# jbrea/BayesianOptimization.jl

Hardware: AMD Instinct MI355X
Metric: acquisition-candidates/sec (N=3000,d=8) (higher is better)
Workload: dtype f64

## Files before the change

### bayesianoptimization.jl_amd/csrc/bohip.hip

```cpp
#include "../../include/bohip.h"
#include "../../include/bohip_paths.h"
#include "../../include/bohip_fit.h"
#include "../../include/bohip_qei.h"
#include "../../include/bohip_acq.h"
#include "../../include/bohip_kg.h"
#include "../../include/bohip_mes.h"
#include "../../include/bohip_ens.h"
#include "../../include/bohip_ens_grad.h"
#include "../../include/bohip_con.h"
#include "../../include/bohip_mo.h"
#include "../../include/bohip_loo.h"
#include "../../include/bohip_loo_batch.h"
#include "../../include/bohip_rep.h"
#include "kernels_linalg.hip"
#include "kernels_loo.hip"
#include "kernels_rep.hip"
#include "kernels_chol.hip"
#include "kernels_exec.hip"
#include "kernels_score.hip"
#include "kernels_batch.hip"
#include "kernels_sample.hip"
#include "kernels_qei.hip"
#include "kernels_kg.hip"
#include "kernels_mes.hip"
// ... 307 lines not shown
    for (DBuf<double>* b : {&g->dX, &g->dy, &g->dL, &g->dW, &g->dWT, &g->dS, &g->dalpha, &g->dr, &g->dt, &g->dApp, &g->dchol_idl}) b->release();
    g->dchol_flags.release();
    g->dinvr.release();
    g->ex_T = 0;
    return 0;
}
static size_t chol_flag_words(int T);
static size_t chol_abort_word(int T);
static int upload_site_weights(bohip_gp* g) {
    HIPCHK(g->dinvr.reserve(std::max<size_t>(1, (size_t)std::max(g->cap, g->n)), g->stream));
    if (g->n > 0) HIPCHK(hipMemcpyAsync(g->dinvr, g->hinvr.data(), (size_t)g->n * 8, hipMemcpyHostToDevice, g->stream));
    return 0;
}
static int refuse_weighted(const bohip_gp* g, const char* who) {
    if (!g || !g->weighted) return 0;
    return fail(BOHIP_E_UNSUPPORTED, std::string(who) + " does not support a model with replicated sites (bohip_gp_append_sites with reps > 1): "
                                         "its kernels build the covariance with one noise term for every row");
}
static int alloc_model(bohip_gp* g, int64_t cap) {
    free_model(g);
    for (DBuf<double>* b : {&g->dKsT, &g->dVT, &g->dUT, &g->dq, &g->dBV}) b->release();
    g->kst_rows = 0;
    g->cap = cap;
    g->ld = round_up(cap + 1, TILE) + 16;
    const size_t ld = (size_t)g->ld, mat = ld * ld * sizeof(double);
    hipStream_t st = g->stream;
    HIPCHK(g->dX.reserve(std::max<size_t>(1, (size_t)cap * g->d), st));
    HIPCHK(g->dy.reserve(std::max<size_t>(1, (size_t)cap), st));
    for (DBuf<double>* b : {&g->dL, &g->dW, &g->dWT, &g->dS}) HIPCHK(b->reserve(ld * ld, st));
    for (DBuf<double>* b : {&g->dalpha, &g->dr, &g->dt}) HIPCHK(b->reserve(ld + 256, st));
    HIPCHK(g->dApp.reserve((size_t)APP_ROWS * ld, st));
    {
        const size_t Tm = (size_t)(g->ld / TILE) + 1;
        HIPCHK(g->dchol_flags.reserve(chol_flag_words((int)std::min<size_t>(Tm, CHOL_DF_TCAP)), st));
        HIPCHK(g->dchol_idl.reserve(Tm * CH_PANELS * 256, st));
    }
    HIPCHK(hipMemsetAsync(g->dL, 0, mat, g->stream));
    HIPCHK(hipMemsetAsync(g->dW, 0, mat, g->stream));
    HIPCHK(hipMemsetAsync(g->dWT, 0, mat, g->stream));
    HIPCHK(hipMemsetAsync(g->dS, 0, mat, g->stream));
    if (g->n > 0) {
        HIPCHK(hipMemcpyAsync(g->dX, g->hX.data(), (size_t)g->n * g->d * 8, hipMemcpyHostToDevice, g->stream));
        HIPCHK(hipMemcpyAsync(g->dy, g->hy.data(), (size_t)g->n * 8, hipMemcpyHostToDevice, g->stream));
    }
    if (g->weighted) CHK(upload_site_weights(g));
    g->stale = true;
    return 0;
}

static int g_bulk_pieces = 4;
static int g_sample_mfma_min = 200;
static int g_path_mfma_min = 24;
static int g_split = 1;
static int g_asc_wg_nmax = 256;
static const double g_asc_first_step = 0.1;
static int g_asc_fold = 1;
static int g_asc_lockstep = 0;
static int g_small_m = 0;
static int g_small_r = -1;
static int g_inv_hi_h = 16;
static int g_chol_df = 1;
static bool g_chol_df_strict = false;
static bool g_chol_df_dump = false;
static int g_chol_df_tmax = 96;
static std::atomic<int> g_chol_df_skip{0}, g_chol_df_backoff{0};
static unsigned long long g_chol_spin_ticks = CH_SPIN_TICKS_DEFAULT;
static int g_chol_exec_patience_us = 1000;
static int g_chol_exec_fill_inv = 1;
static int g_chol_exec_inv_pairs = 0;
static std::atomic<int> g_chol_inv_grp_min{28};
static std::atomic<int> g_chol_inv_g{8};
static int g_chol_nsf = 3;
static int g_chol_exec_urgent = -1;
static int g_chol_exec_second = 1;
static int g_small_zero_copy = 1;
static int g_chol_exec_nbu = 2;
static int g_chol_exec_fast = -1;
static int g_chol_exec_pairs = -1;
static int g_chol_exec_wgs = -1;
static int g_append_alpha_inc = 1;
static int64_t g_chunk_rows_forced = 0;
static int g_prune_m = -1;
static int g_pa_order = 1;
static int launch_gemm_nt(bohip_gp* g, const GemmNTParams& p, int batch = 1, hipStream_t st = nullptr, bool hi = false) {
    if (p.mt <= 0 || p.nt64 <= 0 || p.kc <= 0 || batch <= 0) return 0;
    if (hi) hipLaunchKernelGGL(k_gemm_nt_hi, dim3(p.mt * p.nt64, batch), dim3(GEMM_THREADS_8), glds3_lds_bytes<4>(), st ? st : g->stream, p);
    else hipLaunchKernelGGL(k_gemm_nt, dim3(p.mt * p.nt64, batch), dim3(GEMM_THREADS_8), glds3_lds_bytes<4>(), st ? st : g->stream, p);
    HIPCHK(hipGetLastError());
    return 0;
}

static int device_cus();
static void read_dev_knobs() {
#if BOHIP_DEV_KNOBS
    struct Knob { const char* name; int* v; int lo, hi; };
    static int chunk_rows = 0, dump = 0;
    const Knob knobs[] = {
        {"BOHIP_CHOL_DF_TMAX", &g_chol_df_tmax, 0, CHOL_DF_TCAP}, {"BOHIP_INV_HI_H", &g_inv_hi_h, 0, 1 << 20},
        {"BOHIP_CHOL_EXEC_PAIRS", &g_chol_exec_pairs, -1, 64},
        {"BOHIP_CHOL_EXEC_URGENT", &g_chol_exec_urgent, 1, 1 << 20}, {"BOHIP_CHOL_NSF", &g_chol_nsf, 1, CH_NSF_MAX},
        {"BOHIP_CHOL_EXEC_PATIENCE_US", &g_chol_exec_patience_us, 0, 1 << 30}, {"BOHIP_CHOL_EXEC_FILL_INV", &g_chol_exec_fill_inv, 0, 1},
        {"BOHIP_CHOL_EXEC_INV_PAIRS", &g_chol_exec_inv_pairs, 0, 1}, {"BOHIP_CHOL_EXEC_WGS", &g_chol_exec_wgs, 1, 1 << 20},
        {"BOHIP_CHOL_EXEC_FAST", &g_chol_exec_fast, -1, 1 << 20},
        {"BOHIP_CHOL_EXEC_SECOND", &g_chol_exec_second, 0, 1}, {"BOHIP_SMALL_ZERO_COPY", &g_small_zero_copy, 0, 1}, {"BOHIP_CHOL_EXEC_NBU", &g_chol_exec_nbu, 0, 16}, {"BOHIP_CHUNK_ROWS", &chunk_rows, 0, 1 << 30},
        {"BOHIP_PRUNE_M", &g_prune_m, -1, 1 << 16}, {"BOHIP_PA_ORDER", &g_pa_order, 0, 1},
        {"BOHIP_APPEND_ALPHA_INC", &g_append_alpha_inc, 0, 1}, {"BOHIP_BULK_PIECES", &g_bulk_pieces, 0, 8}, {"BOHIP_SPLIT", &g_split, 0, 1},
        {"BOHIP_SMALL_R", &g_small_r, 0, SMALL_MAX}, {"BOHIP_SMALL_M", &g_small_m, 0, 1 << 20}, {"BOHIP_CHOL_DF_DUMP", &dump, 0, 1},
    };
    for (const Knob& k : knobs)
        if (const char* e = getenv(k.name)) *k.v = std::min(k.hi, std::max(k.lo, atoi(e)));
    g_chunk_rows_forced = chunk_rows;
    g_chol_df_dump = dump != 0;
#endif
}

template <class Setup>
static int once_per_device(bool (&done)[64], int device, Setup&& setup) {
    if (done[device & 63]) return 0;
    CHK(setup());
    done[device & 63] = true;
    return 0;
}

static int kernel_setup_of_this_device() {
    HIPCHK(hipFuncSetAttribute((const void*)k_potf2_inv, hipFuncAttributeMaxDynamicSharedMemorySize, POTF2_LDS_BYTES));
    HIPCHK(hipFuncSetAttribute((const void*)k_gemm_nt, hipFuncAttributeMaxDynamicSharedMemorySize, glds3_lds_bytes<4>()));
    HIPCHK(hipFuncSetAttribute((const void*)k_trigemm_sq, hipFuncAttributeMaxDynamicSharedMemorySize, glds3_lds_bytes<4>()));
    HIPCHK(hipFuncSetAttribute((const void*)k_trigemm_sq_pa, hipFuncAttributeMaxDynamicSharedMemorySize, glds3_lds_bytes<4>()));
    HIPCHK(hipFuncSetAttribute((const void*)k_trigemm_rows, hipFuncAttributeMaxDynamicSharedMemorySize, RS_LDS_BYTES));
    HIPCHK(hipFuncSetAttribute((const void*)k_batch_cond<true>, hipFuncAttributeMaxDynamicSharedMemorySize, BATCH_LDS_MAX));
    HIPCHK(hipFuncSetAttribute((const void*)k_batch_cond<false>, hipFuncAttributeMaxDynamicSharedMemorySize, BATCH_LDS_MAX));
    HIPCHK(hipFuncSetAttribute((const void*)k_chol_chain, hipFuncAttributeMaxDynamicSharedMemorySize, CH_LDS_BYTES));
    HIPCHK(hipFuncSetAttribute((const void*)k_gemm_nt_hi, hipFuncAttributeMaxDynamicSharedMemorySize, glds3_lds_bytes<4>()));
    HIPCHK(hipFuncSetAttribute((const void*)k_chol_exec, hipFuncAttributeMaxDynamicSharedMemorySize, glds3_lds_bytes<4>()));
    HIPCHK(hipFuncSetAttribute((const void*)k_trimv_stream<TRIMV_D>, hipFuncAttributeMaxDynamicSharedMemorySize, trimv_lds_bytes(TRIMV_D)));
    HIPCHK(hipFuncSetAttribute((const void*)k_path_mfma<true>, hipFuncAttributeMaxDynamicSharedMemorySize, (int)path_mfma_lds_bytes(DMAX)));
    HIPCHK(hipFuncSetAttribute((const void*)k_path_mfma<false>, hipFuncAttributeMaxDynamicSharedMemorySize, (int)path_mfma_lds_bytes(DMAX)));
    HIPCHK(hipFuncSetAttribute((const void*)k_kg<true>, hipFuncAttributeMaxDynamicSharedMemorySize, (int)kg_lds_bytes(KG_RMAX)));
    HIPCHK(hipFuncSetAttribute((const void*)k_kg<false>, hipFuncAttributeMaxDynamicSharedMemorySize, (int)kg_lds_bytes(KG_RMAX)));
    if (const char* e = getenv("BOHIP_CHOL_DATAFLOW")) g_chol_df = atoi(e);
    if (const char* e = getenv("BOHIP_CHOL_SPIN_US")) g_chol_spin_ticks = 100ull * (unsigned long long)std::max(1, atoi(e));
    if (const char* e = getenv("BOHIP_CHOL_INV_G")) g_chol_inv_g = std::min(64, std::max(0, atoi(e)));
    if (const char* e = getenv("BOHIP_CHOL_INV_GRP_MIN")) g_chol_inv_grp_min = std::max(0, atoi(e));
    if (const char* e = getenv("BOHIP_ASC_WG_NMAX")) g_asc_wg_nmax = std::max(0, atoi(e));
    if (const char* e = getenv("BOHIP_ASC_LOCKSTEP")) { g_asc_lockstep = atoi(e) == 1; g_asc_fold = atoi(e) != 2; }
    if (const char* e = getenv("BOHIP_SAMPLE_MFMA_MIN")) g_sample_mfma_min = std::max(1, atoi(e));
    g_chol_df_strict = getenv("BOHIP_CHOL_DF_STRICT") != nullptr;
    read_dev_knobs();
    return 0;
}
static int one_time_kernel_setup() {
    static bool done[64] = {false};
    int dev = 0;
    HIPCHK(hipGetDevice(&dev));
    return once_per_device(done, dev, kernel_setup_of_this_device);
}

static int launch_rows_trimv(bohip_gp* g, const double* W, int64_t N0, const double* rows, int P, double* out, int upper);
static int compute_alpha(bohip_gp* g) {
    const int64_t N = g->n;
    g->alpha_inc_run = 0;
    hipLaunchKernelGGL(k_sub_mean, dim3((N + 255) / 256), dim3(256), 0, g->stream, g->dy, g->beta, N, g->dr);
    HIPCHK(hipGetLastError());
    CHK(launch_rows_trimv(g, g->dW, N, g->dr, 1, g->dt, 0));
    CHK(launch_rows_trimv(g, g->dWT, N, g->dt, 1, g->dalpha, 1));
    HIPCHK(hipMemcpyAsync(g->dW + N * g->ld, g->dalpha, (size_t)N * 8, hipMemcpyDeviceToDevice, g->stream));
    return 0;
}

static int check_info(bohip_gp* g) {
    int local = 0;
    int* const pw = g->hpin ? g->pin.words + 1 : &local;
    HIPCHK(hipMemcpyAsync(pw, g->dinfo, sizeof(int), hipMemcpyDeviceToHost, g->stream));
    HIPCHK(hipStreamSynchronize(g->stream));
    const int info = *pw;
    if (info != 0) {
        g->pivot = info;
        g->stale = true;
        return fail(BOHIP_E_NOTPD, "kernel matrix not positive definite at pivot " + std::to_string(info));
    }
    g->pivot = 0;
    return 0;
}

static int inverse_level(bohip_gp* g, hipStream_t st, int t0, int nt, int h) {
    const int64_t ld = g->ld, base = (int64_t)t0 * TILE * (ld + 1);
    const int pairs = (nt + 2 * h - 1) / (2 * h);
    const int64_t zs = (int64_t)2 * h * TILE * (ld + 1);
// ... 841 lines not shown
    if (grew) HIPCHK(hipMemsetAsync(g->dVT, 0, n * 8, g->stream));
    return 0;
}
static int ensure_xs(bohip_gp* g, int64_t R) {
    HIPCHK(g->dXs.reserve(std::max<size_t>(1, (size_t)R * g->d), g->stream));
    return 0;
}

struct PassDims { int64_t N, Npad, R, Rpad, ld; int T; };
static int row_tiles(const bohip_gp* g) { return (int)(round_up(g->n + 1, TILE) / TILE); }
static PassDims pass_dims(const bohip_gp* g, int64_t R) {
    const int T = row_tiles(g);
    return PassDims{g->n, (int64_t)T * TILE, R, round_up(R, TILE) + TILE, g->ld, T};
}
struct SplitPlan { int kz = 0, nsl = 0; };
enum class Route { Small, Split, Pruned, WholeK };
struct PassPlan {
    PassDims dm{};
    Route route = Route::WholeK;
    SplitPlan sp;
    int prune_m = 0;
    int64_t chunk = 0;
    int dq_tiles() const { return route == Route::WholeK || route == Route::Pruned ? dm.T : 0; }
};

template <int DT>
static void launch_kstar(bohip_gp* g, const double* dXs, int64_t r0, int64_t r1, int64_t Npad, const KernelHyper& hp, const KstarParts* kp) {
    const int rb = r1 - r0 <= 32 && !kp ? 2 : 16;
    dim3 grid((Npad + 255) / 256, (r1 - r0 + rb - 1) / rb);
    if (kp)
        LAUNCH_FAM(fam_low(hp), (k_kstar<DT, true, true>), (k_kstar<DT, false, true>), grid, dim3(256), 0, g->stream, g->dX, g->n, Npad, dXs,
                   r0, r1, hp, g->dKsT, g->ld, rb, *kp);
    else
        LAUNCH_FAM(fam_low(hp), (k_kstar<DT, true>), (k_kstar<DT, false>), grid, dim3(256), 0, g->stream, g->dX, g->n, Npad, dXs, r0, r1, hp,
                   g->dKsT, g->ld, rb, KstarParts{});
}

static void trigemm_pieces(int T, int64_t alpha_row, std::vector<int>& out) {
    struct P { double cost; int code; };
    std::vector<P> ps;
    for (int rt = 0; rt < T; ++rt) {
        const int64_t live = alpha_row + 1 - (int64_t)rt * TILE;
        if (live <= TILE / 2) ps.push_back({(rt + 0.5) / 2.0, rt | PIECE_UPPER_SOLO << 16});
        else ps.push_back({rt + 1.0, rt | PIECE_WHOLE << 16});
    }
    std::stable_sort(ps.begin(), ps.end(), [](const P& a, const P& b) { return a.cost > b.cost; });
    out.clear();
    for (const P& q : ps) out.push_back(q.code);
}
static int ensure_pieces(bohip_gp* g, int T, int64_t alpha_row) {
    if (g->pieces_T == T && g->pieces_alpha == alpha_row && g->dpieces) return 0;
    std::vector<int> ps;
    trigemm_pieces(T, alpha_row, ps);
    if (T > 65535) return fail(BOHIP_E_UNSUPPORTED, "too many row tiles");
    if (ps.size() > g->dpieces.capacity()) HIPCHK(g->dpieces.reserve(2 * ps.size() + 64, g->stream));
    g->hpieces = ps;
    HIPCHK(hipMemcpyAsync(g->dpieces, g->hpieces.data(), ps.size() * sizeof(int), hipMemcpyHostToDevice, g->stream));
    g->n_pieces = (int)ps.size();
    g->pieces_T = T; g->pieces_alpha = alpha_row;
    return 0;
}

static int ensure_clk(bohip_gp* g) {
    bool grew = false;
    HIPCHK(g->dclk.reserve(2, g->stream, Grow::Exact, &grew));
    if (grew) HIPCHK(hipMemsetAsync(g->dclk, 0, 2 * sizeof(unsigned long long), g->stream));
    return 0;
}
static int launch_trigemm(bohip_gp* g, const PassDims& dm, int64_t r0, int64_t ncand, double* VT, FuseParams fz) {
    const int CT = (int)((ncand + CTILE - 1) / CTILE), n_local = (CT + 7) / 8;
    CHK(ensure_pieces(g, dm.T, dm.N));
    const int NP = g->n_pieces;
    fz.T = dm.T;
    if (g->timing) {
        CHK(ensure_clk(g));
        fz.clk = g->dclk;
    }
    hipLaunchKernelGGL(k_trigemm_sq, dim3(8 * n_local * NP), dim3(GEMM_THREADS_8), glds3_lds_bytes<4>(), g->stream, g->dW, g->ld,
                       g->dKsT, g->ld, g->dpieces, NP, CT, dm.N, g->dq, dm.Rpad, g->dmu_raw, r0, VT, g->ld, fz);
    HIPCHK(hipGetLastError());
    return 0;
}

static int launch_kstar_any(bohip_gp* g, const double* dXs, int64_t r0, int64_t r1, int64_t Npad, const KernelHyper& hp,
                            const KstarParts* kp = nullptr) {
    dispatch_dt(g->d, [&](auto dt) { launch_kstar<decltype(dt)::value>(g, dXs, r0, r1, Npad, hp, kp); });
    HIPCHK(hipGetLastError());
    return 0;
}

static int launch_gemm_u(bohip_gp* g, const PassDims& dm, int CT) {
    GemmNTParams p{};
    p.A = g->dVT; p.lda = dm.ld; p.B = g->dWT; p.ldb = dm.ld; p.C = g->dUT; p.ldc = dm.ld;
    p.mt = CT; p.nt64 = 2 * dm.T; p.kc = dm.T * (TILE / KC); p.alpha = 1.0; p.beta = 0.0; p.klo_from_n = 1;
    return launch_gemm_nt(g, p);
}

struct ChunkV { double* VT = nullptr; int64_t row_stride = 0; };
template <class Finish>
static int64_t chunk_pass(bohip_gp* g, const PassPlan& pl, const double* dXs, const KernelHyper& hp, ChunkV v, bool want_u, const FuseParams& fz, Finish&& finish) {
    const PassDims& dm = pl.dm;
    int64_t chunks = 0;
    for (int64_t r0 = 0; r0 < dm.R; r0 += pl.chunk, ++chunks) {
        const int64_t r1 = std::min(dm.R, r0 + pl.chunk);
        t_begin(g, "kstar");
        CHK(launch_kstar_any(g, dXs, r0, r1, dm.Npad, hp));
        t_end(g);
        t_begin(g, v.VT ? "trigemm_sq+V" : "trigemm_sq");
        CHK(launch_trigemm(g, dm, r0, r1 - r0, v.VT ? v.VT + r0 * v.row_stride : nullptr, fz));
        t_end(g);
        if (want_u) {
            t_begin(g, "gemm_U");
            CHK(launch_gemm_u(g, dm, (int)((r1 - r0 + TILE - 1) / TILE)));
            t_end(g);
        }
        CHK(finish(r0, r1));
    }
    return chunks;
}
static int no_finish(int64_t, int64_t) { return 0; }

static int ensure_small_counters(bohip_gp* g) {
    bool grew = false;
    HIPCHK(g->dgparts.reserve((size_t)SMALL_MAX * 16 * (2 * DMAX), g->stream));
    HIPCHK(g->dgcount.reserve(SMALL_MAX, g->stream, Grow::Exact, &grew));
    if (grew) HIPCHK(hipMemsetAsync(g->dgcount, 0, SMALL_MAX * sizeof(unsigned), g->stream));
    return 0;
}
static bool split_applicable(const bohip_gp* g);
static int64_t small_limit(const bohip_gp* g) {
    if (g_small_r >= 0) return g_small_r;
    if (split_applicable(g)) return std::min<int64_t>(SMALL_MAX, std::max<int64_t>(16, (20 + 260000 / std::max<int64_t>(g->n, 1)) / 16 * 16));
    return std::min<int64_t>(SMALL_MAX, 90 + 300000 / std::max<int64_t>(g->n, 1));
}
static int64_t path_R(const bohip_gp* g, int64_t R) { return std::max(R, g->batch_hint); }
#ifdef BOHIP_SMALL_TRACE
static unsigned long long* g_small_trace = nullptr;
extern "C" int bohip_debug_small_trace_read(unsigned long long* out) {
    if (!g_small_trace) return -1;
    return hipMemcpy(out, g_small_trace, 8192 * 16 * 8, hipMemcpyDeviceToHost) == hipSuccess ? 0 : -2;
}
#endif
template <int DT, int G>
static void launch_small_pass(bohip_gp* g, const SmallCommon& sc, const SmallCommon& scu, const SmallV& sv, const SmallU* su, const KernelHyper& hp,
                              int npass) {
    const bool lo = fam_low(hp);
    LAUNCH_FAM(lo, (k_small_v<DT, G, true>), (k_small_v<DT, G, false>), dim3((unsigned)sc.ntiles, (unsigned)npass), dim3(SP_THREADS), 0,
               g->stream, sc, sv, hp);
    if (su) {
        if (DT == 64 && su->sv.ap.acq == ACQ_LOGEI)
            LAUNCH_FAM(lo, (k_small_u_logei64<true>), (k_small_u_logei64<false>), dim3((unsigned)sc.ntiles, (unsigned)npass), dim3(SP_THREADS), 0,
                       g->stream, scu, *su, hp);
        else
            LAUNCH_FAM(lo, (k_small_u<DT, G, true>), (k_small_u<DT, G, false>), dim3((unsigned)sc.ntiles, (unsigned)npass), dim3(SP_THREADS), 0,
                       g->stream, scu, *su, hp);
    }
}
template <int DT>
static void launch_small_pass_g(bohip_gp* g, int G, const SmallCommon& sc, const SmallCommon& scu, const SmallV& sv, const SmallU* su,
                                const KernelHyper& hp, int npass) {
    if constexpr (DT <= 16) {
        if (G == 1) return launch_small_pass<DT, 1>(g, sc, scu, sv, su, hp, npass);
        if (G == 2) return launch_small_pass<DT, 2>(g, sc, scu, sv, su, hp, npass);
        if (G == 3) return launch_small_pass<DT, 3>(g, sc, scu, sv, su, hp, npass);
    }
    launch_small_pass<DT, 4>(g, sc, scu, sv, su, hp, npass);
}
struct AscPass {
    const SmallFold* fold = nullptr;
// ... 144 lines not shown
    std::stable_sort(out.begin(), out.end(), [](int a, int b) {
        return 8 * (a & 0xffff) + ((a >> 16) & 1) * 4 > 8 * (b & 0xffff) + ((b >> 16) & 1) * 4;
    });
    return out;
}
static int rows_halves_from(const std::vector<int>& hv, int t0) {
    int n = 0;
    while (n < (int)hv.size() && (hv[n] & 0xffff) >= t0) ++n;
    return n;
}
static int launch_trigemm_rows(bohip_gp* g, const double* KsT, const int* halves, int NH, const int* list, const unsigned* cnt,
                               int cnt_max, double* q, int64_t ldq, double* mu, int groups = 0, const PruneFinish* pf = nullptr,
                               unsigned* arrive = nullptr) {
    if (NH <= 0 || cnt_max <= 0) return 0;
    RowsParams rp{};
    rp.W = g->dW; rp.ldw = g->ld; rp.KsT = KsT; rp.ldk = g->ld; rp.list = list; rp.cnt = cnt; rp.cnt_max = cnt_max;
    rp.halves = halves; rp.NH = NH; rp.G = groups > 0 ? groups : (cnt_max + RS_COLS - 1) / RS_COLS;
    rp.alpha_row = g->n; rp.q = q; rp.ldq = ldq; rp.mu = mu;
    if (pf) { rp.finish = 1; rp.arrive = arrive; rp.pf = *pf; }
    hipLaunchKernelGGL(k_trigemm_rows, dim3((unsigned)(8 * ((NH + 7) / 8) * rp.G)), dim3(RS_THREADS), RS_LDS_BYTES, g->stream, rp);
    HIPCHK(hipGetLastError());
    return 0;
}
static int launch_trigemm_on(bohip_gp* g, const double* KsT, const int* pieces, int NP, int CT, double* q, int64_t ldq, double* mu_raw,
                             FuseParams fz) {
    const int n_local = (CT + 7) / 8;
    if (NP <= 0 || CT <= 0) return 0;
    if (g->timing && g->dclk) fz.clk = g->dclk;
    hipLaunchKernelGGL(k_trigemm_sq, dim3(8 * n_local * NP), dim3(GEMM_THREADS_8), glds3_lds_bytes<4>(), g->stream, g->dW, g->ld, KsT,
                       g->ld, pieces, NP, CT, g->n, q, ldq, mu_raw, (int64_t)0, nullptr, g->ld, fz);
    HIPCHK(hipGetLastError());
    return 0;
}
static std::vector<int> phase_a_jobs(const std::vector<int>& pieces, int m) {
    std::vector<int> out;
    for (int c : pieces)
        if ((c & 0xffff) < m) { out.push_back((c & 0xffff) | 1 << 16); out.push_back(c & 0xffff); }
    std::stable_sort(out.begin(), out.end(), [](int a, int b) {
        return 8 * (a & 0xffff) + (a >> 16) * 4 > 8 * (b & 0xffff) + (b >> 16) * 4;
    });
    if (g_pa_order == 1) std::rotate(out.begin(), out.begin() + out.size() / 3, out.begin() + 2 * (out.size() / 3));
    return out;
}
static int launch_phase_a(bohip_gp* g, const double* KsT, const int* jobs, int NJOBS, int CT, double* q, int64_t ldq) {
    const int n_local = (CT + 7) / 8;
    if (NJOBS <= 0 || CT <= 0) return 0;
    hipLaunchKernelGGL(k_trigemm_sq_pa, dim3(8 * n_local * NJOBS), dim3(GEMM_THREADS_8), glds3_lds_bytes<4>(), g->stream, g->dW, g->ld,
                       KsT, g->ld, jobs, CT, q, ldq, g->timing && g->dclk ? g->dclk : nullptr);
    HIPCHK(hipGetLastError());
    return 0;
}
static int pruned_pass(bohip_gp* g, const double* dXs, const PassPlan& pl, const AcqParams& ap, Best* d_best, int64_t best_off,
                       double* ub_host = nullptr, bool long_form = false) {
    CHK(one_time_kernel_setup());
    {
        bool grew = false;
        HIPCHK(g->hprune_stat.reserve(16, g->stream, Grow::Exact, &grew));
        if (grew) g->hprune_stat[0] = 0u;
    }
    const int64_t N = pl.dm.N, Npad = pl.dm.Npad, R = pl.dm.R, Rpad = pl.dm.Rpad, ld = pl.dm.ld;
    const int T = pl.dm.T, m = pl.prune_m;
    const int64_t P = Npad / 64;
    CHK(ensure_pieces(g, T, N));
    if (m >= T) return fail(BOHIP_E_STATE, "pruned pass: the prefix holds the alpha row");
    for (int c : g->hpieces)
        if ((c & 0xffff) < m && c >> 16 != PIECE_WHOLE) return fail(BOHIP_E_STATE, "pruned pass: a half piece in the prefix");
    layout::PrunedWs ws;
    auto lay = [&](const void* base) {
        return layout::pruned(base, (size_t)Rpad * ld, (size_t)2 * T * Rpad, (size_t)Rpad, PRUNE_K1, (size_t)2 * P * Rpad, 5 * g->hpieces.size() + 8, &ws);
    };
    bool fresh = false;
    HIPCHK(g->dpr.reserve(lay(nullptr), g->stream, Grow::Exact, &fresh));
    lay(g->dpr);
    double *ks2 = ws.ks, *q2 = ws.q2, *mu2 = ws.mu2, *ub = ws.ub;
    int *l1 = ws.l1, *l2 = ws.l2, *mark = ws.mark, *pcs = ws.pcs;
    const KstarParts kp{g->dW + N * ld, ws.parts, Rpad};
    g->pr_ks_len = (size_t)((char*)ws.q2 - (char*)ws.ks);
    unsigned* cnt = ws.cnt;
    Best* rec = static_cast<Best*>(ws.rec);
    if (g->timing) CHK(ensure_clk(g));
    g->score_launches = 1;
    const KernelHyper hp = make_hyper(g);
    t_begin(g, "kstar");
    CHK(launch_kstar_any(g, dXs, 0, R, Npad, hp, &kp));
    t_end(g);
    std::vector<int> pa, pb;
    for (int c : g->hpieces) ((c & 0xffff) < m ? pa : pb).push_back(c);
    const std::vector<int> ph = phase_a_jobs(g->hpieces, m);
    const std::vector<int> hv = rows_halves(g->hpieces);
    const int nh = rows_halves_from(hv, m);
    std::vector<int> both = pa;
    both.insert(both.end(), pb.begin(), pb.end());
    both.insert(both.end(), hv.begin(), hv.end());
    both.insert(both.end(), ph.begin(), ph.end());
    if (fresh || g->hpr_pieces != both || g->pr_pieces_at != pcs) {
        g->pr_pieces_at = pcs;
        g->hpr_pieces = both;
        HIPCHK(hipMemcpyAsync(pcs, g->hpr_pieces.data(), both.size() * sizeof(int), hipMemcpyHostToDevice, g->stream));
    }
    const double sigma2 = std::exp(2.0 * g->logsig);
    const int k1 = (int)std::min<int64_t>(PRUNE_K1, R);
    t_begin(g, "trigemm_sq");
    FuseParams fz{};
    fz.T = T;
    CHK(launch_phase_a(g, g->dKsT, pcs + pa.size() + pb.size() + hv.size(), (int)ph.size(), (int)((R + CTILE - 1) / CTILE), g->dq, Rpad));
    PruneBound bd{};
    bd.parts = kp.parts; bd.P = P; bd.ldp = Rpad; bd.Npad = Npad; bd.q = g->dq; bd.ldq = Rpad; bd.R = R; bd.m = m;
    bd.sigma2 = sigma2; bd.beta = g->beta; bd.ap = ap; bd.ub = ub;
    hipLaunchKernelGGL(k_prune_bound, dim3((unsigned)((R + 63) / 64)), dim3(64), 0, g->stream, bd);
    if (ub_host) {
        t_end(g);
        HIPCHK(hipGetLastError());
        HIPCHK(hipMemcpyAsync(ub_host, ub, (size_t)R * 8, hipMemcpyDeviceToHost, g->stream));
        HIPCHK(hipStreamSynchronize(g->stream));
        return 0;
    }
    static_assert(PRUNE_R_MAX <= (int64_t)SELECT_THREADS * SELECT_PER, "k_prune_select holds the whole batch in one workgroup");
    hipLaunchKernelGGL(k_prune_select, dim3(1), dim3(SELECT_THREADS), 0, g->stream, (const double*)ub, R, k1, l1, mark, cnt, rec);
    HIPCHK(hipGetLastError());
    PruneFinish pf{};
    pf.q = g->dq; pf.ldq = Rpad; pf.q2 = q2; pf.ldq2 = Rpad; pf.mu2 = mu2; pf.m = m; pf.T = T; pf.sigma2 = sigma2; pf.beta = g->beta;
    pf.ap = ap; pf.rec = rec;
    const int* hvd = pcs + pa.size() + pb.size();
    pf.ub = ub; pf.mark = mark; pf.R = R; pf.cnt2 = cnt + 1; pf.best_off = (long long)best_off;
    pf.list = l1; pf.cnt = cnt; pf.list2 = l2; pf.best_out = d_best; pf.stat = g->hprune_stat;
    CHK(launch_trigemm_rows(g, g->dKsT, hvd, nh, l1, cnt, k1, q2, Rpad, mu2, 0, &pf, cnt + PRUNE_ARRIVE));
    const int64_t cap = R - k1;
    pf.list = l2; pf.cnt = cnt + 1; pf.list2 = nullptr;
    if (cap > 0 && !long_form) {
        CHK(launch_trigemm_rows(g, g->dKsT, hvd, nh, l2, cnt + 1, INT_MAX, q2, Rpad, mu2, PRUNE_R2_GROUPS, &pf, cnt + PRUNE_ARRIVE + 1));
    } else if (cap > 0) {
        if (cap > PRUNE_ROWS_CAP) {
            hipLaunchKernelGGL(k_prune_gather, dim3((unsigned)cap), dim3(256), 0, g->stream, (const int*)l2, (const unsigned*)(cnt + 1),
                               (const double*)g->dKsT, ld, Npad, ks2, PRUNE_ROWS_CAP, cnt + 2);
            fz.live = cnt + 2;
            CHK(launch_trigemm_on(g, ks2, pcs + pa.size(), (int)pb.size(), (int)((cap + CTILE - 1) / CTILE), q2, Rpad, mu2, fz));
        }
        CHK(launch_trigemm_rows(g, g->dKsT, hvd, nh, l2, cnt + 1, (int)std::min<int64_t>(cap, PRUNE_ROWS_CAP), q2, Rpad, mu2));
        hipLaunchKernelGGL(k_prune_finish, dim3(1), dim3(256), 0, g->stream, pf);
        HIPCHK(hipGetLastError());
    }
    t_end(g);
    return 0;
}

constexpr int PRUNE_BACKOFF = 31;
static bool prune_wanted(bohip_gp* g, int64_t R) {
    if (g->prune_skip > 0) { --g->prune_skip; return false; }
    g->prune_seen = 0u;
    if (g->hprune_stat) {
        const unsigned n2 = __atomic_load_n(g->hprune_stat.get(), __ATOMIC_RELAXED);
        g->prune_seen = n2;
        if ((int64_t)n2 > R / 8) {
            __atomic_store_n(g->hprune_stat.get(), 0u, __ATOMIC_RELAXED);
            g->prune_skip = PRUNE_BACKOFF - 1;
            g->prune_retry = true;
            return false;
        }
    }
    return true;
}

enum class Prune { No, Value, Probe };
struct RouteWants { bool small = true, split = true; Prune prune = Prune::No; };
static constexpr RouteWants WHOLE_K_ONLY{false, false, Prune::No};
static PassPlan choose_route(bohip_gp* g, int64_t R, RouteWants w) {
    PassPlan pl;
// ... 2706 lines not shown
    if (!g || R <= 0 || !Xs || !q_out || !mu_out || path < 0 || path > 3) return fail(BOHIP_E_ARG, "bad arguments");
    HIPCHK(hipSetDevice(g->device));
    if (g->n == 0) return fail(BOHIP_E_STATE, "model has no observations");
    CHK(ensure_fresh(g));
    CHK(ensure_xs(g, R));
    CHK(ensure_score_scratch(g, R));
    if (R > chunk_rows(g, R)) return fail(BOHIP_E_UNSUPPORTED, "more than one K*' chunk");
    CHK(one_time_kernel_setup());
    const PassDims dm = pass_dims(g, R);
    const int64_t N = dm.N, Npad = dm.Npad, Rpad = round_up(R, TILE);
    const int T = dm.T;
    CHK(ensure_pieces(g, T, N));
    const std::vector<int> hv = rows_halves(g->hpieces);
    HIPCHK(hipMemcpyAsync(g->dXs, Xs, (size_t)R * g->d * 8, hipMemcpyHostToDevice, g->stream));
    CHK(launch_kstar_any(g, g->dXs, 0, R, Npad, make_hyper(g)));
    std::vector<double> q((size_t)2 * T * Rpad), mu((size_t)Rpad);
    if (path == 0) {
        CHK(launch_trigemm_on(g, g->dKsT, g->dpieces, g->n_pieces, (int)((R + CTILE - 1) / CTILE), g->dq, Rpad, g->dmu_raw, FuseParams{}));
        HIPCHK(hipMemcpyAsync(q.data(), g->dq, q.size() * 8, hipMemcpyDeviceToHost, g->stream));
        HIPCHK(hipMemcpyAsync(mu.data(), g->dmu_raw, mu.size() * 8, hipMemcpyDeviceToHost, g->stream));
        HIPCHK(hipStreamSynchronize(g->stream));
        for (int t = 0; t < 2 * T; ++t) std::memcpy(q_out + (size_t)t * R, q.data() + (size_t)t * Rpad, (size_t)R * 8);
        std::memcpy(mu_out, mu.data(), (size_t)R * 8);
        return 0;
    }
    if (path == 3) {
        const int m = prune_tiles(T);
        if (m <= 0 || m >= T) return fail(BOHIP_E_UNSUPPORTED, "no pruning at this size");
        const std::vector<int> ph = phase_a_jobs(g->hpieces, m);
        int* dj = nullptr;
        HIPCHK(hipMalloc(&dj, ph.size() * sizeof(int)));
        hipMemcpyAsync(dj, ph.data(), ph.size() * sizeof(int), hipMemcpyHostToDevice, g->stream);
        hipMemsetAsync(g->dq, 0, q.size() * 8, g->stream);
        const int rc = launch_phase_a(g, g->dKsT, dj, (int)ph.size(), (int)((R + CTILE - 1) / CTILE), g->dq, Rpad);
        hipMemcpyAsync(q.data(), g->dq, q.size() * 8, hipMemcpyDeviceToHost, g->stream);
        const hipError_t e = hipStreamSynchronize(g->stream);
        hipFree(dj);
        if (rc != 0) return rc;
        if (e != hipSuccess) return fail(BOHIP_E_HIP, hipGetErrorString(e));
        for (int t = 0; t < 2 * T; ++t) std::memcpy(q_out + (size_t)t * R, q.data() + (size_t)t * Rpad, (size_t)R * 8);
        std::memset(mu_out, 0, (size_t)R * 8);
        return 0;
    }
    std::vector<int> list((size_t)R);
    for (int64_t i = 0; i < R; ++i) list[i] = (int)(R - 1 - i);
    const unsigned n = (unsigned)R;
    char* d = nullptr;
    const size_t o_q = 0, o_mu = o_q + q.size() * 8, o_l = o_mu + mu.size() * 8, o_h = o_l + list.size() * 4, o_c = o_h + hv.size() * 4;
    HIPCHK(hipMalloc(&d, o_c + 16));
    int rc = 0;
    hipMemcpyAsync(d + o_l, list.data(), list.size() * 4, hipMemcpyHostToDevice, g->stream);
    hipMemcpyAsync(d + o_h, hv.data(), hv.size() * 4, hipMemcpyHostToDevice, g->stream);
    hipMemcpyAsync(d + o_c, &n, 4, hipMemcpyHostToDevice, g->stream);
    rc = launch_trigemm_rows(g, g->dKsT, (const int*)(d + o_h), (int)hv.size(), (const int*)(d + o_l), (const unsigned*)(d + o_c), (int)R,
                             (double*)(d + o_q), Rpad, (double*)(d + o_mu), path == 2 ? 1 : 0);
    hipMemcpyAsync(q.data(), d + o_q, q.size() * 8, hipMemcpyDeviceToHost, g->stream);
    hipMemcpyAsync(mu.data(), d + o_mu, mu.size() * 8, hipMemcpyDeviceToHost, g->stream);
    const hipError_t e = hipStreamSynchronize(g->stream);
    hipFree(d);
    if (rc != 0) return rc;
    if (e != hipSuccess) return fail(BOHIP_E_HIP, hipGetErrorString(e));
    for (int t = 0; t < 2 * T; ++t)
        for (int64_t i = 0; i < R; ++i) q_out[(size_t)t * R + list[i]] = q[(size_t)t * Rpad + i];
    for (int64_t i = 0; i < R; ++i) mu_out[list[i]] = mu[i];
    return 0;
}
int64_t bohip_debug_prune_stat(bohip_gp* g) {
    if (!g || !g->hprune_stat) return -1;
    return (int64_t)__atomic_load_n(g->hprune_stat.get(), __ATOMIC_RELAXED);
}
int bohip_debug_prune_round2_form(bohip_gp* g, int form) {
    if (!g || form < -1 || form > 1) return fail(BOHIP_E_ARG, "bad arguments");
    g->prune_r2_form = form;
    return 0;
}
int bohip_debug_kstar_poison(bohip_gp* g) {
    if (!g) return fail(BOHIP_E_ARG, "bad arguments");
    HIPCHK(hipSetDevice(g->device));
    if (g->dKsT) HIPCHK(hipMemsetAsync(g->dKsT, 0xff, (size_t)(g->kst_rows + TILE) * g->ld * 8, g->stream));
    if (g->dpr && g->pr_ks_len) HIPCHK(hipMemsetAsync(g->dpr, 0xff, std::min(g->pr_ks_len, g->dpr.capacity()), g->stream));
    HIPCHK(hipStreamSynchronize(g->stream));
    return 0;
}
int bohip_debug_set_chol_inv_g(int g_new) {
    return g_chol_inv_g.exchange(std::min(64, std::max(0, g_new)));
}
int bohip_debug_exec_throughput(bohip_gp* g, unsigned qmask, int hot, int wgs, double* ms_out, double* gflop_out) {
    if (!g || !ms_out || g->n == 0) return BOHIP_E_ARG;
    hipSetDevice(g->device);
    CHK(one_time_kernel_setup());
    const int T = row_tiles(g);
    if (T <= 3) return BOHIP_E_UNSUPPORTED;
    std::vector<ExTask> all, run;
    int qb[EX_NQ + 1], qb2[EX_NQ + 1];
    exec_task_list(g->dL, g->dS, g->dW, g->dWT, g->dchol_flags, g->ld, T, g_chol_nsf, g_chol_inv_g, all, qb);
    double fl = 0.0;
    qb2[0] = 0;
    for (int qi = 0; qi < EX_NQ; ++qi) {
        if ((qmask >> qi) & 1u)
            for (int i = qb[qi]; i < qb[qi + 1]; ++i) {
                ExTask t = all[i];
                for (int d = 0; d < EX_NDEP; ++d) { t.dep_idx[d] = EX_NONE; t.dep_want[d] = 0; }
                t.sig_idx[0] = t.sig_idx[1] = EX_NONE;
                t.kc_split = 0; t.dep2_idx[0] = t.dep2_idx[1] = EX_NONE;
                if (hot && (qi == EX_QBULK || qi == EX_QWAVE)) { t.A = g->dS; t.B = g->dS + (int64_t)TILE * g->ld; }
                fl += 2.0 * TILE * CTILE * KC * t.kc;
                run.push_back(t);
            }
        qb2[qi + 1] = (int)run.size();
    }
    if (run.empty()) return BOHIP_E_ARG;
    ExTask* dt = nullptr;
    HIPCHK(hipMalloc(&dt, run.size() * sizeof(ExTask)));
    HIPCHK(hipMemcpy(dt, run.data(), run.size() * sizeof(ExTask), hipMemcpyHostToDevice));
    HIPCHK(hipMemsetAsync(g->dchol_flags, 0, chol_flag_words(T) * sizeof(unsigned), g->stream));
    ExQueues q{};
    q.tasks = dt;
    for (int i = 0; i <= EX_NQ; ++i) q.qbeg[i] = qb2[i];
    q.flags = g->dchol_flags;
    q.abort = g->dchol_flags + chol_abort_word(T);
    q.heads = q.abort + 1;
    q.ld = g->ld;
    q.spin_ticks = g_chol_spin_ticks;
    const int exec_wgs = wgs > 0 ? wgs : std::max(2, std::min(g_chol_exec_wgs > 0 ? g_chol_exec_wgs : 1 << 20, 2 * std::max(1, device_cus() - (9 + g_chol_nsf + 6))));
    q.nurgent = std::max(1, std::min(exec_wgs / 8, g_chol_exec_urgent > 0 ? g_chol_exec_urgent : (T >= 56 ? 16 : 32)));
    const int pairs_ = g_chol_exec_pairs == 0 ? 0 : 1;
        q.stride[0] = 1; q.stride[1] = 1; q.stride[2] = pairs_ ? 2 : 1; q.stride[EX_QBULK] = pairs_ >= 2 ? 2 * std::min(pairs_, 4) : (pairs_ ? 2 : 1);
    q.stride[EX_QROWS] = q.stride[EX_QWAVE] = g_chol_exec_inv_pairs ? 2 : 1;
    q.fill_inv = g_chol_exec_fill_inv;
    q.patience_ticks = (unsigned)g_chol_exec_patience_us * 100u;
    hipEvent_t e0, e1;
    HIPCHK(hipEventCreate(&e0)); HIPCHK(hipEventCreate(&e1));
    HIPCHK(hipEventRecord(e0, g->stream));
    hipLaunchKernelGGL(k_chol_exec, dim3(exec_wgs), dim3(GEMM_THREADS_8), glds3_lds_bytes<4>(), g->stream, q);
    HIPCHK(hipGetLastError());
    HIPCHK(hipEventRecord(e1, g->stream));
    HIPCHK(hipEventSynchronize(e1));
    float ms = 0.f;
    HIPCHK(hipEventElapsedTime(&ms, e0, e1));
    hipEventDestroy(e0); hipEventDestroy(e1);
    hipFree(dt);
    *ms_out = ms;
    if (gflop_out) *gflop_out = fl * 1e-9;
    g->stale = true;
    g->w_done = false;
    return 0;
}
#if BOHIP_CHOL_TRACE
int bohip_debug_chol_trace_read(unsigned long long* out, int64_t n_words) {
    return hipMemcpyFromSymbol(out, HIP_SYMBOL(bohip::g_chol_trace), (size_t)n_words * 8) == hipSuccess ? 0 : -3;
}
int bohip_debug_exec_trace_read(unsigned long long* out, int64_t n_words) {
    return hipMemcpyFromSymbol(out, HIP_SYMBOL(bohip::g_ex_trace), (size_t)n_words * 8) == hipSuccess ? 0 : -3;
}
#endif
#if BOHIP_TRACE
int bohip_debug_trace_read(unsigned long long* out, int64_t n_words) {
    return hipMemcpyFromSymbol(out, HIP_SYMBOL(bohip::g_trace), (size_t)n_words * 8) == hipSuccess ? 0 : -3;
}
int bohip_debug_phase_read(unsigned long long* out, int64_t n_words) {
    return hipMemcpyFromSymbol(out, HIP_SYMBOL(bohip::g_phase), (size_t)n_words * 8) == hipSuccess ? 0 : -3;
}
#endif
}
```

### bayesianoptimization.jl_amd/csrc/kernels_score.hip

```cpp
#include "gemm_core.h"
#include "acq_log.h"

namespace bohip {

template <bool LOW>
__device__ __forceinline__ double cov_from_r_fast(int fam, double sigma2, double r) {
    if constexpr (LOW) {
        return matern_lo_k(fam, sigma2, r);
    } else {
        if (fam == FAM_M52) {
            const double R = sqrt(r), s = sqrt(5.0) * R;
            return sigma2 * (1.0 + s + 5.0 / 3.0 * r) * exp(-s);
        }
        return sigma2 * exp(-0.5 * r);
    }
}

struct KstarParts {
    const double* alpha;
    double* parts;
    int64_t ldp;
};
template <int DT, bool LOW>
__device__ __forceinline__ double kstar_value(const double (&xj)[DT], const double (&w)[DT], const double* xs, bool live, int fam,
// ... 13 lines not shown
    x = __longlong_as_double((long long)((unsigned long long)hi[0] << 32 | lo[0]));
    y = __longlong_as_double((long long)((unsigned long long)hi[1] << 32 | lo[1]));
}
template <int BIT>
__device__ __forceinline__ double halve_sum(double a, double b, int lane) {
    const bool up = lane & BIT;
    return (up ? b : a) + __shfl_xor(up ? a : b, BIT);
}
__device__ __forceinline__ void group_sum4(const double* p, int lane, double& sm, double& sa) {
    double x0, y0, x1, y1;
    swap32(p[0], p[2], x0, y0);
    swap32(p[1], p[3], x1, y1);
    sm = halve_sum<16>(x0 + y0, x1 + y1, lane);
    sa = halve_sum<16>(fabs(x0) + fabs(y0), fabs(x1) + fabs(y1), lane);
}
__device__ __forceinline__ double wave_finish(double s) {
    s += __shfl_xor(s, 2);
    s += __shfl_xor(s, 1);
    return s;
}

template <int DT, bool LOW, bool PARTS = false>
__global__ __launch_bounds__(256) void k_kstar(const double* __restrict__ X, int64_t N, int64_t Npad,
                                               const double* __restrict__ Xs, int64_t r_begin, int64_t r_end,
                                               KernelHyper hp, double* __restrict__ KsT, int64_t ldk, int rb, KstarParts kp) {
    __shared__ double xs_l[16 * DT];
    const int d = hp.d;
    const int64_t j = blockIdx.x * 256 + threadIdx.x;
    const int64_t r0 = r_begin + (int64_t)blockIdx.y * rb;
    const int64_t r1 = min(r0 + rb, r_end);
    for (int t = threadIdx.x; t < rb * DT; t += 256) {
        const int64_t r = r0 + t / DT;
        const int k = t % DT;
        xs_l[t] = (r < r1 && k < d) ? Xs[r * d + k] : 0.0;
    }
    double xj[DT], w[DT];
#pragma unroll
    for (int k = 0; k < DT; ++k) {
        xj[k] = (k < d && j < N) ? X[j * d + k] : 0.0;
        w[k] = k < d ? hp.il2[k] : 0.0;
    }
    __syncthreads();
    if (j >= Npad) return;
    const int nc = (int)(r1 - r0);
    if constexpr (PARTS) {
        const double aj = kp.alpha[j];
        const int lane = threadIdx.x & 63;
        double um[2], ua[2], tm0 = 0.0, ta0 = 0.0;
#pragma unroll
        for (int g = 0; g < 4; ++g) {
            double p[4];
#pragma unroll
            for (int i = 0; i < 4; ++i) {
                const int c = 4 * g + i;
                p[i] = 0.0;
                if (c < nc) {
                    const double v = kstar_value<DT, LOW>(xj, w, xs_l + c * DT, j < N, hp.fam, hp.sigma2);
                    KsT[(r0 + c - r_begin) * ldk + j] = v;
                    p[i] = aj * v;
                }
            }
            double tm, ta;
            group_sum4(p, lane, tm, ta);
            if (g & 1) {
                um[g >> 1] = halve_sum<8>(tm0, tm, lane);
                ua[g >> 1] = halve_sum<8>(ta0, ta, lane);
            } else {
                tm0 = tm;
                ta0 = ta;
            }
            __builtin_amdgcn_sched_barrier(0);
        }
        const double sm = wave_finish(halve_sum<4>(um[0], um[1], lane)), sa = wave_finish(halve_sum<4>(ua[0], ua[1], lane));
        const int c = 8 * ((lane >> 2) & 1) + 4 * ((lane >> 3) & 1) + 2 * (lane >> 5) + ((lane >> 4) & 1);
        if ((lane & 3) < 2 && c < nc) {
            const int64_t P = Npad >> 6;
            kp.parts[((int64_t)(lane & 1) * P + (j >> 6)) * kp.ldp + (r0 + c - r_begin)] = (lane & 1) ? sa : sm;
        }
    } else {
        for (int c = 0; c < nc; ++c) {
            const double v = kstar_value<DT, LOW>(xj, w, xs_l + c * DT, j < N, hp.fam, hp.sigma2);
            KsT[(r0 + c - r_begin) * ldk + j] = v;
        }
    }
}

template <int DT, bool LOW>
__global__ __launch_bounds__(256) void k_post_cov(const double* __restrict__ Xs, int64_t R, KernelHyper hp,
                                                  const double* __restrict__ VV, int64_t ldv,
                                                  double* __restrict__ cov, int64_t ldc) {
    const int d = hp.d;
    const int64_t s = blockIdx.x * 256 + threadIdx.x;
    if (s >= R) return;
    double xs[DT];
#pragma unroll
    for (int k = 0; k < DT; ++k) xs[k] = (k < d) ? Xs[s * d + k] : 0.0;
    const int64_t r0 = (int64_t)blockIdx.y * 16, r1 = min(R, r0 + 16);
    for (int64_t r = r0; r < r1; ++r) {
        double rr = 0.0;
#pragma unroll
        for (int k = 0; k < DT; ++k)
            if (k < d) {
                const double t = Xs[r * d + k] - xs[k];
                rr += hp.il2[k] * (t * t);
            }
        const double vv = (r >= s) ? VV[r * ldv + s] : VV[s * ldv + r];
        cov[r * ldc + s] = cov_from_r_fast<LOW>(hp.fam, hp.sigma2, rr) - vv;
    }
}

struct AcqParams {
    int acq;
    double p0, p1;
};
struct FuseParams {
    unsigned* tile_cnt;
    unsigned* total_cnt;
    Best* tile_best;
    int tiles_total;
    int T;
    int64_t R_total;
    double sigma2, beta;
    AcqParams ap;
    double *mu_out, *var_out, *score_out;
    Best* best_out;
    long long best_off;
    unsigned long long* clk;
    const unsigned* live;
};
__device__ void trigemm_fused_finish(const FuseParams& fz, int tile_g, int T, const double* q_part, int64_t ldq,
                                     const double* mu_raw);

#if BOHIP_TRACE
__device__ unsigned long long g_trace[6 * 8192];
#endif
constexpr int PIECE_WHOLE = 0, PIECE_UPPER_SOLO = 3;

__device__ __forceinline__ double sq_step(double s, double v) { return s + v * v; }
__device__ __forceinline__ double sq_tree(double s) {
    s += __shfl_xor(s, 8);
    s += __shfl_xor(s, 16);
    s += __shfl_xor(s, 32);
    return s;
}

__device__ __forceinline__ void trigemm_job(int rt, int mode, int ct, const double* __restrict__ W, int64_t ldw,
                                            const double* __restrict__ KsT, int64_t ldk, int NP, int64_t alpha_row,
                                            double* __restrict__ q_part, int64_t ldq, double* __restrict__ mu_raw, int64_t r_off,
                                            double* __restrict__ VT, int64_t ldv, const FuseParams& fz, double* smem, int tid) {
    constexpr int NJ = 4, CW = CTILE;
    double acc[8][NJ];
#pragma unroll
    for (int i = 0; i < 8; ++i)
#pragma unroll
        for (int j = 0; j < NJ; ++j) acc[i][j] = 0.0;
    const int64_t row_base = (int64_t)rt * TILE;
    const int active_rows = (int)min((int64_t)(mode == PIECE_WHOLE ? TILE : TILE / 2), alpha_row + 1 - row_base);
    const int tri_kc = rt * (TILE / KC);
    const int kc_end = mode == PIECE_WHOLE ? (rt + 1) * (TILE / KC) : tri_kc + 4;
    gemm_tile_loop_glds3_ks<NJ, BOHIP_ABL, true>(W + row_base * ldw, ldw, KsT + (int64_t)ct * CW * ldk, ldk, 0, kc_end, smem, acc,
                                                 active_rows, tri_kc, tid);
    const int lane = tid & 63, wave = tid >> 6, wr = (wave & 3) >> 1, wc = wave & 1;
    __syncthreads();
    double* red = smem;
    const bool rows_mine = mode == PIECE_WHOLE || wr == 0;
    if (wave < 4) {
// ... 1048 lines not shown
```

Measured before the change: 29.47 million.

## Add column-major K* kernel with per-wave LDS transpose for pruned pass

Adds k_kstar_cols, which assigns each lane one candidate row and walks 64 training columns held in LDS. It accumulates the alpha-weighted partial sums (signed and absolute) in registers and transposes 16-column pieces through a per-wave LDS tile, so KsT is written as coalesced double2 stores. The pruned scoring pass now uses it for d<=16, replacing the previous kstar launch that needed cross-lane reductions for the partial sums. In exchange it adds a per-dimension template dispatch, a new shape knob, and a debug entry point for comparing the kernel forms.

```diff
diff --git a/bayesianoptimization.jl_amd/csrc/bohip.hip b/bayesianoptimization.jl_amd/csrc/bohip.hip
--- a/bayesianoptimization.jl_amd/csrc/bohip.hip
+++ b/bayesianoptimization.jl_amd/csrc/bohip.hip
@@ -413,6 +413,7 @@
 static int64_t g_chunk_rows_forced = 0;
 static int g_prune_m = -1;
 static int g_pa_order = 1;
+static int g_kcols_shape = 0;
 static int launch_gemm_nt(bohip_gp* g, const GemmNTParams& p, int batch = 1, hipStream_t st = nullptr, bool hi = false) {
     if (p.mt <= 0 || p.nt64 <= 0 || p.kc <= 0 || batch <= 0) return 0;
     if (hi) hipLaunchKernelGGL(k_gemm_nt_hi, dim3(p.mt * p.nt64, batch), dim3(GEMM_THREADS_8), glds3_lds_bytes<4>(), st ? st : g->stream, p);
@@ -434,7 +435,7 @@
         {"BOHIP_CHOL_EXEC_INV_PAIRS", &g_chol_exec_inv_pairs, 0, 1}, {"BOHIP_CHOL_EXEC_WGS", &g_chol_exec_wgs, 1, 1 << 20},
         {"BOHIP_CHOL_EXEC_FAST", &g_chol_exec_fast, -1, 1 << 20},
         {"BOHIP_CHOL_EXEC_SECOND", &g_chol_exec_second, 0, 1}, {"BOHIP_SMALL_ZERO_COPY", &g_small_zero_copy, 0, 1}, {"BOHIP_CHOL_EXEC_NBU", &g_chol_exec_nbu, 0, 16}, {"BOHIP_CHUNK_ROWS", &chunk_rows, 0, 1 << 30},
-        {"BOHIP_PRUNE_M", &g_prune_m, -1, 1 << 16}, {"BOHIP_PA_ORDER", &g_pa_order, 0, 1},
+        {"BOHIP_PRUNE_M", &g_prune_m, -1, 1 << 16}, {"BOHIP_PA_ORDER", &g_pa_order, 0, 1}, {"BOHIP_KCOLS_SHAPE", &g_kcols_shape, 0, 3},
         {"BOHIP_APPEND_ALPHA_INC", &g_append_alpha_inc, 0, 1}, {"BOHIP_BULK_PIECES", &g_bulk_pieces, 0, 8}, {"BOHIP_SPLIT", &g_split, 0, 1},
         {"BOHIP_SMALL_R", &g_small_r, 0, SMALL_MAX}, {"BOHIP_SMALL_M", &g_small_m, 0, 1 << 20}, {"BOHIP_CHOL_DF_DUMP", &dump, 0, 1},
     };
@@ -1442,9 +1443,29 @@
     return 0;
 }
 
+constexpr int KCOLS_SHAPES[] = {4, 2, 3, 1};
+template <int D = 1, class F>
+static void dispatch_d16(int d, F&& f) {
+    if constexpr (D <= KC_DMAX) {
+        if (d == D) f(std::integral_constant<int, D>{});
+        else dispatch_d16<D + 1>(d, f);
+    }
+}
+static void launch_kstar_cols(bohip_gp* g, const double* dXs, int64_t R, int64_t Npad, const KernelHyper& hp, const KstarParts& kp) {
+    const int nw = KCOLS_SHAPES[g_kcols_shape];
+    const dim3 grid((unsigned)(Npad / 64), (unsigned)((R + 64 * nw - 1) / (64 * nw)));
+    dispatch_d16(g->d, [&](auto dd) {
+        constexpr int D = decltype(dd)::value;
+        LAUNCH_FAM(fam_low(hp), (k_kstar_cols<D, true>), (k_kstar_cols<D, false>), grid, dim3(64 * nw), (64 * D + 64) * 8 + nw * KC_TILE_BYTES,
+                   g->stream, g->dX, g->n, Npad, dXs, R, hp, g->dKsT, g->ld, kp.alpha, kp.parts, kp.ldp);
+    });
+}
+
 static int launch_kstar_any(bohip_gp* g, const double* dXs, int64_t r0, int64_t r1, int64_t Npad, const KernelHyper& hp,
-                            const KstarParts* kp = nullptr) {
-    dispatch_dt(g->d, [&](auto dt) { launch_kstar<decltype(dt)::value>(g, dXs, r0, r1, Npad, hp, kp); });
+                            const KstarParts* kp = nullptr, bool cols = false) {
+    if (cols && (r0 != 0 || !kp)) return fail(BOHIP_E_STATE, "k_kstar_cols: every candidate, with the partial sums");
+    if (cols && g->d <= KC_DMAX) launch_kstar_cols(g, dXs, r1, Npad, hp, *kp);
+    else dispatch_dt(g->d, [&](auto dt) { launch_kstar<decltype(dt)::value>(g, dXs, r0, r1, Npad, hp, kp); });
     HIPCHK(hipGetLastError());
     return 0;
 }
@@ -1755,7 +1776,7 @@
     g->score_launches = 1;
     const KernelHyper hp = make_hyper(g);
     t_begin(g, "kstar");
-    CHK(launch_kstar_any(g, dXs, 0, R, Npad, hp, &kp));
+    CHK(launch_kstar_any(g, dXs, 0, R, Npad, hp, &kp, true));
     t_end(g);
     std::vector<int> pa, pb;
     for (int c : g->hpieces) ((c & 0xffff) < m ? pa : pb).push_back(c);
@@ -4628,6 +4649,37 @@
     HIPCHK(hipStreamSynchronize(g->stream));
     return 0;
 }
+int bohip_debug_kstar_forms(bohip_gp* g, const double* Xs, int64_t R, int form, double* ks_out, double* parts_out, double* alpha_out,
+                            int64_t* npad_out) {
+    if (!g || R <= 0 || !Xs || !npad_out || form < 0 || form > 2) return fail(BOHIP_E_ARG, "bad arguments");
+    HIPCHK(hipSetDevice(g->device));
+    if (g->n == 0) return fail(BOHIP_E_STATE, "model has no observations");
+    CHK(ensure_fresh(g));
+    CHK(ensure_xs(g, R));
+    CHK(ensure_score_scratch(g, R));
+    if (R > chunk_rows(g, R)) return fail(BOHIP_E_UNSUPPORTED, "more than one K*' chunk");
+    const PassDims dm = pass_dims(g, R);
+    const int64_t P = dm.Npad / 64;
+    *npad_out = dm.Npad;
+    if (!ks_out) return 0;
+    if (!alpha_out || (form > 0 && !parts_out)) return fail(BOHIP_E_ARG, "bad arguments");
+    double* dparts = nullptr;
+    HIPCHK(hipMalloc(&dparts, (size_t)2 * P * dm.Rpad * 8));
+    hipMemsetAsync(dparts, 0xff, (size_t)2 * P * dm.Rpad * 8, g->stream);
+    hipMemsetAsync(g->dKsT, 0xff, (size_t)(g->kst_rows + TILE) * g->ld * 8, g->stream);
+    hipMemcpyAsync(g->dXs, Xs, (size_t)R * g->d * 8, hipMemcpyHostToDevice, g->stream);
+    const KstarParts kp{g->dW + dm.N * dm.ld, dparts, dm.Rpad};
+    const int rc = launch_kstar_any(g, g->dXs, 0, R, dm.Npad, make_hyper(g), form ? &kp : nullptr, form == 2);
+    hipMemcpy2DAsync(ks_out, (size_t)dm.Npad * 8, g->dKsT, (size_t)g->ld * 8, (size_t)dm.Npad * 8, (size_t)R, hipMemcpyDeviceToHost, g->stream);
+    if (form)
+        hipMemcpy2DAsync(parts_out, (size_t)R * 8, dparts, (size_t)dm.Rpad * 8, (size_t)R * 8, (size_t)2 * P, hipMemcpyDeviceToHost, g->stream);
+    hipMemcpyAsync(alpha_out, kp.alpha, (size_t)dm.Npad * 8, hipMemcpyDeviceToHost, g->stream);
+    const hipError_t e = hipStreamSynchronize(g->stream);
+    hipFree(dparts);
+    if (rc != 0) return rc;
+    if (e != hipSuccess) return fail(BOHIP_E_HIP, hipGetErrorString(e));
+    return 0;
+}
 int bohip_debug_set_chol_inv_g(int g_new) {
     return g_chol_inv_g.exchange(std::min(64, std::max(0, g_new)));
 }
diff --git a/bayesianoptimization.jl_amd/csrc/kernels_score.hip b/bayesianoptimization.jl_amd/csrc/kernels_score.hip
--- a/bayesianoptimization.jl_amd/csrc/kernels_score.hip
+++ b/bayesianoptimization.jl_amd/csrc/kernels_score.hip
@@ -119,6 +119,110 @@
             const double v = kstar_value<DT, LOW>(xj, w, xs_l + c * DT, j < N, hp.fam, hp.sigma2);
             KsT[(r0 + c - r_begin) * ldk + j] = v;
         }
+    }
+}
+
+constexpr int KC_LD = 18;
+constexpr int KC_TILE_BYTES = 64 * KC_LD * 8;
+constexpr int KC_DMAX = 16;
+__device__ __forceinline__ void kc_add(double aj, double v, double& sm, double& sa) {
+#pragma clang fp contract(off)
+    const double p = aj * v;
+    sm += p;
+    sa += fabs(p);
+}
+__device__ __forceinline__ void kc_wave_sync() {
+    __builtin_amdgcn_fence(__ATOMIC_RELEASE, "wavefront");
+    __builtin_amdgcn_wave_barrier();
+    __builtin_amdgcn_fence(__ATOMIC_ACQUIRE, "wavefront");
+}
+
+constexpr int KC_UNROLL = 2;
+template <int D, bool LOW>
+__global__ __launch_bounds__(256) void k_kstar_cols(const double* __restrict__ X, int64_t N, int64_t Npad,
+                                                    const double* __restrict__ Xs, int64_t R, KernelHyper hp,
+                                                    double* __restrict__ KsT, int64_t ldk,
+                                                    const double* __restrict__ alpha, double* __restrict__ parts, int64_t ldp) {
+    static_assert(D >= 1 && D <= KC_DMAX, "wider models keep k_kstar<DT, LOW, true>");
+    extern __shared__ __align__(16) double kc_lds[];
+    const int nw = blockDim.x >> 6;
+    const int wv = __builtin_amdgcn_readfirstlane((int)(threadIdx.x >> 6)), lane = threadIdx.x & 63;
+    const int64_t P = Npad >> 6, wb = blockIdx.x, j0 = wb * 64;
+    const int jn = (int)min((int64_t)64, max(N - j0, (int64_t)0));
+    double* xb = kc_lds;
+    double* ab = kc_lds + 64 * D;
+    double* tile = ab + 64 + wv * (64 * KC_LD);
+    for (int t = threadIdx.x; t < jn * D; t += blockDim.x) xb[t] = X[j0 * D + t];
+    if ((int)threadIdx.x < jn) ab[threadIdx.x] = alpha[j0 + threadIdx.x];
+    __syncthreads();
+    const int64_t r0 = ((int64_t)blockIdx.y * nw + wv) * 64;
+    if (r0 >= R) return;
+    const int64_t r = r0 + lane;
+    const bool mine = r < R;
+    double xs[D], w[D];
+#pragma unroll
+    for (int k = 0; k < D; ++k) {
+        xs[k] = mine ? Xs[r * D + k] : 0.0;
+        w[k] = hp.il2[k];
+    }
+    const int cl = lane >> 3, h = lane & 7;
+    const double* piece = tile + cl * KC_LD + 2 * h;
+    double* mycol = tile + lane * KC_LD;
+    char* out = reinterpret_cast<char*>(KsT + r0 * ldk + j0);
+    const unsigned row8 = (unsigned)(8 * ldk * 8);
+    const unsigned off = (unsigned)((cl * ldk + 2 * h) * 8);
+    const bool whole = R - r0 >= 64;
+    double sm = 0.0, sa = 0.0;
+    auto walk = [&](auto famc) {
+        constexpr int FAM = decltype(famc)::value;
+        const int fam = FAM < 0 ? hp.fam : FAM;
+        double xn[D], an;
+#pragma unroll
+        for (int k = 0; k < D; ++k) xn[k] = xb[k];
+        an = ab[0];
+#pragma unroll 1
+        for (int q = 0; q < 4; ++q) {
+            const int ni = __builtin_amdgcn_readfirstlane(min(16, max(jn - 16 * q, 0)));
+#pragma unroll KC_UNROLL
+            for (int i = 0; i < ni; ++i) {
+                double xj[D];
+#pragma unroll
+                for (int k = 0; k < D; ++k) xj[k] = xn[k];
+                const double aj = an;
+                const int jx = min(16 * q + i + 1, 63);
+#pragma unroll
+                for (int k = 0; k < D; ++k) xn[k] = xb[jx * D + k];
+                an = ab[jx];
+                const double v = kstar_value<D, LOW>(xj, w, xs, true, fam, hp.sigma2);
+                kc_add(aj, v, sm, sa);
+                mycol[i] = v;
+            }
+            for (int i = ni; i < 16; ++i) mycol[i] = 0.0;
+            kc_wave_sync();
+            double2 val[8];
+#pragma unroll
+            for (int s = 0; s < 8; ++s) val[s] = *reinterpret_cast<const double2*>(piece + s * (8 * KC_LD));
+            if (whole) {
+#pragma unroll
+                for (int s = 0; s < 8; ++s) *reinterpret_cast<double2*>(out + (off + s * row8)) = val[s];
+            } else {
+#pragma unroll
+                for (int s = 0; s < 8; ++s)
+                    if (r0 + 8 * s + cl < R) *reinterpret_cast<double2*>(out + (off + s * row8)) = val[s];
+            }
+            kc_wave_sync();
+            out += 16 * 8;
+        }
+    };
+    if constexpr (LOW) {
+        walk(std::integral_constant<int, -1>{});
+    } else {
+        if (hp.fam == FAM_M52) walk(std::integral_constant<int, FAM_M52>{});
+        else walk(std::integral_constant<int, FAM_SE>{});
+    }
+    if (mine) {
+        parts[wb * ldp + r] = sm;
+        parts[(P + wb) * ldp + r] = sa;
     }
 }
 
```

After: 30.16 million, median of 4. No clear change (+2.3%).
